# showlab/VideoSwap

Measured on AMD Instinct MI355X. Metric: denoised frames/sec, 16-frame 512x512 clip @ 50 DDIM steps (end to end: inversion + CFG sampling), higher is better.
Workload: dtype f16; 1 GPU; BASELINE.json configs[1]: 16-frame 512x512 clip, SD-1.5 UNet3D + AnimateDiff motion modules, 50-step DDIM inversion (B=1) + 50-step CFG-7.5 DDIM sampling (B=2), 1 clip per GPU per step; launch=eager, parallelism=clip-parallel x1

## Files before the change

### videoswap_amd/csrc/gemm.hip

```cpp
#include "gemm_common.h"
#include "prof.h"
#include <algorithm>
#include <cstdlib>
#include <stdlib.h>
#include <string.h>

using namespace vsxg;

static long tile_tune() { return vsxg::gemm_option("tile_tune"); }
static long force_tile() { return tile_tune() & 15; }
static bool tune_deep() { return (tile_tune() & 16) != 0; }
static int tune_splits() { return (int)((tile_tune() >> 8) & 15); }

namespace {


#ifdef VSX_GEMM_TIMING
#define TSTAMP(i) do { const long t_now = (long)clock64(); t_seg[i] += t_now - t_last; t_last = t_now; } while (0)
#else
#define TSTAMP(i) do { } while (0)
#endif

template <int BM, int BN, int WAVES_M, int WAVES_N, bool SWAP, int NSTAGE>
__global__ __launch_bounds__(WAVES_M* WAVES_N * 64) void gemm_kernel(const GemmParams p) {
    constexpr int PREFETCH = NSTAGE - 1;
    constexpr int NW = WAVES_M * WAVES_N;
    constexpr int WM = BM / WAVES_M, WN = BN / WAVES_N;
    constexpr int TM = WM / 32, TN = WN / 32;
    constexpr int A_BLKS = BM / 8, B_BLKS = BN / 8;
    static_assert(A_BLKS % NW == 0, "A blocks must split evenly over the waves");
    constexpr int GA = A_BLKS / NW;
    constexpr int GB_LO = B_BLKS / NW, GB_HI = (B_BLKS + NW - 1) / NW;
    constexpr int N_HI = B_BLKS - GB_LO * NW;
    constexpr int STAGE = (BM + BN) * 128;

    extern __shared__ __attribute__((aligned(16))) unsigned char smem[];

    const int tid = threadIdx.x;
    const int lane = tid & 63;
    const int wave = __builtin_amdgcn_readfirstlane(tid >> 6);
    const int wr = wave / WAVES_N, wc = wave % WAVES_N;
    const int l31 = lane & 31, hi = lane >> 5;
#ifdef VSX_GEMM_TIMING
    const long t_begin = (long)clock64();
#endif

    int tile_n, tile_m, split;
    if (p.xcd_gm > 0) {
        const int xcd = blockIdx.x & 7, local = blockIdx.x >> 3;
        const int gm = p.xcd_gm;
        const int RB = p.tiles_m / gm;
        const int CB = (p.tiles_n * (p.splitk > 1 ? p.splitk : 1)) / (8 / gm);
        const int lr = local % RB;
        const int np = (xcd / gm) * CB + local / RB;
        tile_m = (xcd % gm) * RB + lr;
        tile_n = np % p.tiles_n;
        split = np / p.tiles_n;
    } else {
        int wg = blockIdx.x;
        const int nwg = gridDim.x, q = nwg >> 3, r = nwg & 7;
        const int xcd = wg & 7, local = wg >> 3;
        wg = (xcd < r ? xcd * (q + 1) : r * (q + 1) + (xcd - r) * q) + local;
        tile_n = wg % p.tiles_n;
        tile_m = wg / p.tiles_n;
        split = p.splitk > 1 ? (int)blockIdx.z : 0;
    }
    const long m0 = (long)tile_m * BM;
    const long n0 = p.geglu ? (long)tile_n * (BN / 2) : (long)tile_n * BN;

    const int z = (p.splitk > 1 || p.xcd_gm > 0) ? 0 : (int)blockIdx.z;
    const int z0 = z / p.batch1, z1 = z - z0 * p.batch1;
    const half_t* Ab = p.A + z0 * p.a_bs0 + z1 * p.a_bs1;
    const half_t* Bb = p.B + z0 * p.b_bs0 + z1 * p.b_bs1;

    constexpr int OOB_OFF = (int)0x80000000;
    const int lrow = lane >> 3;
    const int pslot = lane & 7;
    const int kofs_e = (pslot ^ (lrow >> 1)) * 8;
    const int kofs_o = (pslot ^ (4 | (lrow >> 1))) * 8;

    const __amdgpu_buffer_rsrc_t rsrcA =
        __builtin_amdgcn_make_buffer_rsrc(const_cast<half_t*>(Ab), 0, (int)p.a_bytes, 0x00020000);
    const __amdgpu_buffer_rsrc_t rsrcA2 =
        __builtin_amdgcn_make_buffer_rsrc(const_cast<half_t*>(p.A2 ? p.A2 : p.A), 0, (int)p.a2_bytes, 0x00020000);
    const __amdgpu_buffer_rsrc_t rsrcB =
        __builtin_amdgcn_make_buffer_rsrc(const_cast<half_t*>(Bb), 0, (int)p.b_bytes, 0x00020000);

// ... 9 lines not shown
        a_ok[i] = m < p.M;
        a_h0[i] = 0; a_w0[i] = 0; a_ibase[i] = 0;
        a_kofs[i] = ((wave * GA + i) & 1) ? kofs_o : kofs_e;
        va[i] = a_ok[i] ? (int)((m * p.lda + a_kofs[i]) * 2) : OOB_OFF;
        if (p.a_mode == 1) {
            const long hw = (long)p.Ho * p.Wo;
            const long mm = a_ok[i] ? m : 0;
            const int img = (int)(mm / hw);
            const int rem = (int)(mm - (long)img * hw);
            const int ho = rem / p.Wo;
            a_h0[i] = ho * p.stride - pad;
            a_w0[i] = (rem - ho * p.Wo) * p.stride - pad;
            a_ibase[i] = img * Hs;
        }
    }
    const int gbw = wave < N_HI ? GB_HI : GB_LO;
    const int b_blk0 = wave < N_HI ? wave * GB_HI : N_HI * GB_HI + (wave - N_HI) * GB_LO;
    int vb[GB_HI], b_kofs[GB_HI];
#pragma unroll
    for (int j = 0; j < GB_HI; ++j) {
        const int jr = (b_blk0 + j) * 8 + lrow;
        b_kofs[j] = ((b_blk0 + j) & 1) ? kofs_o : kofs_e;
        long n;
        bool ok;
        if (p.geglu) {
            const long oc = n0 + (jr >> 5) * 16 + (jr & 15);
            ok = oc < p.N;
            n = oc + ((jr & 16) ? p.N : 0);
        } else {
            n = n0 + jr;
            ok = n < p.N;
        }
        vb[j] = (ok && j < gbw) ? (int)((n * p.ldb + b_kofs[j]) * 2) : OOB_OFF;
    }

    const int Ctot = p.C1 + p.C2;
    const int nk = (int)((p.K + BK - 1) / BK);
    const int ktail_from = (int)(p.K - (long)(nk - 1) * BK);
    const bool fast_tap = p.a_mode == 1 && (Ctot % BK == 0) && (p.C1 % BK == 0);
    const int kt_begin = split * p.nk_per;
    const int kt_end = p.splitk > 1 ? min(nk, kt_begin + p.nk_per) : nk;
    int t_kh = 0, t_kw = 0, t_c = 0;
    bool t_second = false, t_dirty = true;
    if (fast_tap && kt_begin > 0) {
        const int k0 = kt_begin * BK;
        const int tap = k0 / Ctot, rem = k0 - tap * Ctot;
        t_kh = tap / p.ks;
        t_kw = tap - t_kh * p.ks;
        t_second = rem >= p.C1;
        t_c = t_second ? rem - p.C1 : rem;
    }

    unsigned char* i_sb = smem;
    bool i_tail = false, i_second = false;
    int i_soffA = 0, i_soffB = 0;
    auto issue_prep = [&](int kt, int stage) {
        unsigned char* sb = smem + stage * STAGE;
        const bool last_tail = (kt == nk - 1) && ktail_from < BK;
        int soffA = kt * (BK * 2), soffB = kt * (BK * 2);
        bool second = false;
        if (p.a_mode == 1) {
            if (fast_tap) {
                if (t_dirty) {
                    const int cs = t_second ? p.C2 : p.C1;
#pragma unroll
                    for (int i = 0; i < GA; ++i) {
                        const int hh = a_h0[i] + t_kh, ww = a_w0[i] + t_kw;
                        const bool ok = a_ok[i] && (unsigned)hh < (unsigned)p.H && (unsigned)ww < (unsigned)p.W;
                        const int hsrc = p.ups ? (hh >> 1) : hh, wsrc = p.ups ? (ww >> 1) : ww;
                        va[i] = ok ? (((a_ibase[i] + hsrc) * Ws + wsrc) * cs + a_kofs[i]) * 2 : OOB_OFF;
                    }
                    t_dirty = false;
                }
                second = t_second;
                soffA = t_c * 2;
                t_c += BK;
                if (t_c >= (t_second ? p.C2 : p.C1)) {
                    t_c = 0;
                    t_dirty = true;
                    if (!t_second && p.C2 > 0) {
                        t_second = true;
                    } else {
                        t_second = false;
                        if (++t_kw == p.ks) { t_kw = 0; ++t_kh; }
                    }
                }
            } else {
#pragma unroll
                for (int i = 0; i < GA; ++i) {
                    const long k = (long)kt * BK + a_kofs[i];
                    const int kk = k < p.K ? (int)k : 0;
                    const int tap = kk / Ctot;
                    const int ci = kk - tap * Ctot;
                    const int kh = tap / p.ks, kw = tap - kh * p.ks;
                    const int hh = a_h0[i] + kh, ww = a_w0[i] + kw;
                    const bool ok = a_ok[i] && k < p.K && (unsigned)hh < (unsigned)p.H && (unsigned)ww < (unsigned)p.W;
                    const int hsrc = p.ups ? (hh >> 1) : hh, wsrc = p.ups ? (ww >> 1) : ww;
                    va[i] = ok ? (((a_ibase[i] + hsrc) * Ws + wsrc) * p.C1 + ci) * 2 : OOB_OFF;
                }
                soffA = 0;
            }
        }
        i_sb = sb; i_tail = last_tail; i_second = second; i_soffA = soffA; i_soffB = soffB;
    };
    constexpr int NPIECE = GA + GB_HI;
    bool i_on = true;
    bool i_gate = true;
    auto issue_piece = [&](const int q) {
        if (!(i_on && i_gate)) return;
        if (q < GA) {
            const int qi = q < GA ? q : 0;
            const int v = (i_tail && a_kofs[qi] >= ktail_from) ? OOB_OFF : va[qi];
            lptr_t dst = (lptr_t)(i_sb + (wave * GA + q) * 1024);
            if (i_second)
                __builtin_amdgcn_raw_ptr_buffer_load_lds(rsrcA2, dst, 16, v, i_soffA, 0, 0);
            else
                __builtin_amdgcn_raw_ptr_buffer_load_lds(rsrcA, dst, 16, v, i_soffA, 0, 0);
        } else {
            const int j = q - GA;
            if (j < gbw) {
                const int jj = j < GB_HI ? j : 0;
                const int v = (i_tail && b_kofs[jj] >= ktail_from) ? OOB_OFF : vb[jj];
                __builtin_amdgcn_raw_ptr_buffer_load_lds(rsrcB, (lptr_t)(i_sb + BM * 128 + (b_blk0 + j) * 1024), 16, v,
                                                         i_soffB, 0, 0);
            }
        }
    };
    auto issue = [&](int kt, int stage) {
        issue_prep(kt, stage);
        i_on = true;
        i_gate = true;
#pragma unroll
        for (int q = 0; q < NPIECE; ++q) issue_piece(q);
    };

    constexpr int NACC = SWAP ? TN : TM, MACC = SWAP ? TM : TN;
    f16v acc[NACC][MACC];
#pragma unroll
    for (int i = 0; i < NACC; ++i)
#pragma unroll
        for (int j = 0; j < MACC; ++j)
#pragma unroll
            for (int r = 0; r < 16; ++r) acc[i][j][r] = 0.f;

    const int swz = (l31 >> 1) & 7;
    const int a_row = (wr * WM + l31) * 128;
    const int b_row = BM * 128 + (wc * WN + l31) * 128;
    int offs[4];
#pragma unroll
    for (int ks = 0; ks < 4; ++ks) offs[ks] = ((ks * 2 + hi) ^ swz) * 16;

    const int nloc = kt_end - kt_begin;
#pragma unroll
    for (int s = 0; s < PREFETCH; ++s)
        if (s < nloc) issue(kt_begin + s, s);

    constexpr bool PRE_RES = SWAP && (NW <= 8) && (TM * TN <= 5);
    constexpr int NRES = TM * TN * 2;
    h4 rpre[PRE_RES ? TM * TN * 4 : 1];
    const half_t* Rb0 = p.residual ? p.residual + z0 * p.r_bs0 + z1 * p.r_bs1 : nullptr;
    const bool pre_res = PRE_RES && Rb0 != nullptr && p.vec4 && !p.geglu && p.splitk <= 1;
    const bool res_late = pre_res && p.rvec8 && (int)n0 + BN <= (int)p.N;
    bool r_inflight = false;
    auto issue_residual = [&]() {
        if constexpr (PRE_RES) {
#pragma unroll
            for (int i = 0; i < TM; ++i) {
                const unsigned m = (unsigned)min((int)m0 + wr * WM + i * 32 + l31, (int)p.M - 1);
#pragma unroll
                for (int j = 0; j < TN; ++j)
#pragma unroll
                    for (int a = 0; a < 2; ++a) {
                        const int nc = (int)n0 + wc * WN + j * 32 + 16 * a + 8 * hi;
                        const uint4 v = *reinterpret_cast<const uint4*>(Rb0 + m * (unsigned)p.ldr + nc);
                        rpre[(i * TN + j) * 4 + 2 * a] = __builtin_bit_cast(h4, make_uint2(v.x, v.y));
                        rpre[(i * TN + j) * 4 + 2 * a + 1] = __builtin_bit_cast(h4, make_uint2(v.z, v.w));
                    }
            }
        }
    };
    const bool res_early = (p.pp_flags & TILE_RES_EARLY) != 0;
    const int kt_r = res_early ? 0 : max(nloc - 1 - PREFETCH, 0);
    bool r_loaded = false;
    auto wait_slab = [&](const int kt) {
        const int later = min(nloc - 1 - kt, PREFETCH - 1);
        if (PRE_RES && r_inflight) {
            if (wave < N_HI) {
                constexpr int G = GA + GB_HI;
                if (PREFETCH >= 3 && later >= 2) wait_vmcnt<2 * G + NRES>();
                else if (PREFETCH >= 2 && later == 1) wait_vmcnt<G + NRES>();
                else wait_vmcnt<NRES>();
            } else {
                constexpr int G = GA + GB_LO;
                if (PREFETCH >= 3 && later >= 2) wait_vmcnt<2 * G + NRES>();
                else if (PREFETCH >= 2 && later == 1) wait_vmcnt<G + NRES>();
                else wait_vmcnt<NRES>();
            }
            return;
        }
        if (wave < N_HI) {
            constexpr int G = GA + GB_HI;
            if (PREFETCH >= 3 && later >= 2) wait_vmcnt<2 * G>();
            else if (PREFETCH >= 2 && later == 1) wait_vmcnt<G>();
            else wait_vmcnt<0>();
        } else {
            constexpr int G = GA + GB_LO;
            if (PREFETCH >= 3 && later >= 2) wait_vmcnt<2 * G>();
            else if (PREFETCH >= 2 && later == 1) wait_vmcnt<G>();
            else wait_vmcnt<0>();
        }
    };
    auto ldfrag = [&](const unsigned char* sb, const int off, h8 (&af)[TM], h8 (&bf)[TN]) {
#pragma unroll
        for (int i = 0; i < TM; ++i) af[i] = *reinterpret_cast<const h8*>(sb + a_row + i * 4096 + off);
#pragma unroll
        for (int j = 0; j < TN; ++j) bf[j] = *reinterpret_cast<const h8*>(sb + b_row + j * 4096 + off);
    };
    auto mma = [&](const h8 (&af)[TM], const h8 (&bf)[TN]) {
#pragma unroll
        for (int i = 0; i < TM; ++i)
#pragma unroll
            for (int j = 0; j < TN; ++j) {
                if constexpr (SWAP)
                    acc[j][i] = __builtin_amdgcn_mfma_f32_32x32x16_f16(bf[j], af[i], acc[j][i], 0, 0, 0);
                else
                    acc[i][j] = __builtin_amdgcn_mfma_f32_32x32x16_f16(af[i], bf[j], acc[i][j], 0, 0, 0);
            }
    };

    auto mma_issue = [&](const h8 (&af)[TM], const h8 (&bf)[TN], const bool gate) {
        i_gate = gate;
#pragma unroll
        for (int i = 0; i < TM; ++i)
#pragma unroll
            for (int j = 0; j < TN; ++j) {
                if constexpr (SWAP)
                    acc[j][i] = __builtin_amdgcn_mfma_f32_32x32x16_f16(bf[j], af[i], acc[j][i], 0, 0, 0);
                else
                    acc[i][j] = __builtin_amdgcn_mfma_f32_32x32x16_f16(af[i], bf[j], acc[i][j], 0, 0, 0);
                if (i * TN + j < NPIECE) issue_piece(i * TN + j);
            }
#pragma unroll
        for (int q = TM * TN; q < NPIECE; ++q) issue_piece(q);
    };

#ifdef VSX_GEMM_TIMING
    long t_seg[4] = {0, 0, 0, 0}, t_last = 0, t_loop0 = 0;
#endif
    constexpr bool PIPE = (NW <= 8) && (TM * TN < 10);
    if constexpr (PIPE) {
        h8 af0[TM], bf0[TN], af1[TM], bf1[TN];
        wait_slab(0);
        __builtin_amdgcn_s_barrier();
        if (PREFETCH < nloc) issue(kt_begin + PREFETCH, PREFETCH & (NSTAGE - 1));
        ldfrag(smem, offs[0], af0, bf0);
        const bool late = NW >= 8 && wave >= NW / 2;
        i_on = false;
#ifdef VSX_GEMM_TIMING
        t_last = t_loop0 = (long)clock64();
#endif
        for (int kt = 0; kt + 1 < nloc; ++kt) {
            const unsigned char* sb = smem + (kt & (NSTAGE - 1)) * STAGE;
            ldfrag(sb, offs[1], af1, bf1);
            __builtin_amdgcn_sched_barrier(0);
            mma_issue(af0, bf0, late);
            __builtin_amdgcn_sched_barrier(0);
            if constexpr (PRE_RES) {
                if (res_late && kt == kt_r) {
                    issue_residual();
                    VSX_VMEM_NOTE(NRES);
                    r_inflight = !res_early;
                    r_loaded = true;
                }
                __builtin_amdgcn_sched_barrier(0);
            }
            ldfrag(sb, offs[2], af0, bf0);
            __builtin_amdgcn_sched_barrier(0);
            mma(af1, bf1);
            __builtin_amdgcn_sched_barrier(0);
            ldfrag(sb, offs[3], af1, bf1);
            __builtin_amdgcn_sched_barrier(0);
            mma(af0, bf0);
            __builtin_amdgcn_sched_barrier(0);
            TSTAMP(0);
            wait_slab(kt + 1);
            __builtin_amdgcn_s_waitcnt(0xC07F);
            TSTAMP(1);
            __builtin_amdgcn_s_barrier();
            TSTAMP(2);
            i_on = kt + 1 + PREFETCH < nloc;
            if (i_on) issue_prep(kt_begin + kt + 1 + PREFETCH, (kt + 1 + PREFETCH) & (NSTAGE - 1));
            ldfrag(smem + ((kt + 1) & (NSTAGE - 1)) * STAGE, offs[0], af0, bf0);
            __builtin_amdgcn_sched_barrier(0);
            mma_issue(af1, bf1, !late);
            __builtin_amdgcn_sched_barrier(0);
            TSTAMP(3);
        }
        if (nloc > 0) {
            const unsigned char* sb = smem + ((nloc - 1) & (NSTAGE - 1)) * STAGE;
            ldfrag(sb, offs[1], af1, bf1);
            mma(af0, bf0);
            ldfrag(sb, offs[2], af0, bf0);
            mma(af1, bf1);
            ldfrag(sb, offs[3], af1, bf1);
            mma(af0, bf0);
            mma(af1, bf1);
        }
    } else {
        const bool late16 = NW >= 16 && ((wave >> 2) & 1);
#ifdef VSX_GEMM_TIMING
        t_last = t_loop0 = (long)clock64();
#endif
        for (int kt = 0; kt < nloc; ++kt) {
            wait_slab(kt);
            TSTAMP(1);
            __builtin_amdgcn_s_barrier();
            TSTAMP(2);
            i_on = kt + PREFETCH < nloc;
            i_gate = true;
            if (i_on) issue_prep(kt_begin + kt + PREFETCH, (kt + PREFETCH) & (NSTAGE - 1));
            if (!late16) {
#pragma unroll
                for (int q = 0; q < NPIECE; ++q) issue_piece(q);
            }
            TSTAMP(3);
            const unsigned char* sb = smem + (kt & (NSTAGE - 1)) * STAGE;
#pragma unroll
            for (int ks = 0; ks < 4; ++ks) {
                h8 af[TM], bf[TN];
                ldfrag(sb, offs[ks], af, bf);
                mma(af, bf);
                if (ks == 0 && late16) {
#pragma unroll
                    for (int q = 0; q < NPIECE; ++q) issue_piece(q);
                }
            }
            TSTAMP(0);
        }
    }

#ifdef VSX_GEMM_TIMING
    long* const t_out = p.ws && p.splitk <= 1 ? reinterpret_cast<long*>(p.ws) + ((long)blockIdx.x * NW + wave) * 8 : nullptr;
    if (lane == 0 && t_out) {
        for (int k = 0; k < 4; ++k) t_out[k] = t_seg[k];
        t_out[4] = t_begin; t_out[5] = t_loop0; t_out[6] = (long)clock64();
    }
#define TSTAMP_END() do { asm volatile("s_waitcnt vmcnt(0)" ::: "memory"); if (lane == 0 && t_out) t_out[7] = (long)clock64(); } while (0)
#else
#define TSTAMP_END() do { } while (0)
#endif
    half_t* Cb = p.C + z0 * p.c_bs0 + z1 * p.c_bs1;
    const half_t* Rb = p.residual ? p.residual + z0 * p.r_bs0 + z1 * p.r_bs1 : nullptr;
    const int Mi = (int)p.M, Ni = (int)p.N;
    const int ldc = (int)p.ldc, ldr = (int)p.ldr;
    const int mb = (int)m0, nb0 = (int)n0;

    if constexpr (SWAP) {
        if (p.splitk > 1) {
            float* wsl = p.ws + (size_t)split * (size_t)Mi * (size_t)Ni;
#pragma unroll
            for (int i = 0; i < TM; ++i) {
                const int m = mb + wr * WM + i * 32 + l31;
                if (m >= Mi) continue;
#pragma unroll
                for (int j = 0; j < TN; ++j)
#pragma unroll
                    for (int g = 0; g < 4; ++g) {
                        const int nb = nb0 + wc * WN + j * 32 + 8 * g + 4 * hi;
                        if (nb + 3 < Ni) {
                            f4v o;
#pragma unroll
                            for (int e = 0; e < 4; ++e) o[e] = acc[j][i][4 * g + e] * p.alpha;
                            *reinterpret_cast<f4v*>(wsl + (size_t)m * Ni + nb) = o;
                        }
                    }
            }
            return;
        }
        constexpr bool PRE_BIAS = (NW <= 8) && (TM * TN <= 5);
        h4 bpre[PRE_BIAS ? TN : 1][4];
        const bool pre_bias = PRE_BIAS && p.bias != nullptr && p.vec8 && !p.geglu;
        if constexpr (PRE_BIAS) {
            if (pre_bias) {
#pragma unroll
                for (int j = 0; j < TN; ++j)
#pragma unroll
                    for (int g = 0; g < 4; ++g) {
                        const int nb = nb0 + wc * WN + j * 32 + 8 * g + 4 * hi;
                        bpre[j][g] = nb + 3 < Ni ? *reinterpret_cast<const h4*>(p.bias + nb) : h4{};
                    }
            }
        }
#pragma unroll
        for (int i = 0; i < TM; ++i) {
            const int m = mb + wr * WM + i * 32 + l31;
// ... 269 lines not shown
    if (p.residual) {
        const h4 b = *reinterpret_cast<const h4*>(p.residual + (size_t)m * p.ldr + nb);
#pragma unroll
        for (int e = 0; e < 4; ++e) acc[e] += (float)b[e];
    }
    h4 pk;
#pragma unroll
    for (int e = 0; e < 4; ++e) pk[e] = (half_t)acc[e];
    *reinterpret_cast<h4*>(p.C + (size_t)m * p.ldc + nb) = pk;
}

inline int plan_splitk(const vsx_gemm_desc* d, long tiles, bool eligible) {
    const long nk = (d->K + BK - 1) / BK;
    if (eligible && tune_splits() > 0) return tune_splits() <= nk ? tune_splits() : (int)nk;
    if (!eligible || tiles >= 160) return 1;
    int s = (int)((256 + tiles - 1) / tiles);
    if (s > 8) s = 8;
    while (s > 1 && nk / s < 12) --s;
    return s;
}

int plan_xcd_grid(const GemmParams& p, const long tiles_m, const int bm, const int bn, const long nbatch) {
    if (nbatch != 1 || gemm_option("xcd_walk") == 0) return 0;
    const int splits = p.splitk > 1 ? p.splitk : 1;
    const long np_total = (long)p.tiles_n * splits;
    if ((tiles_m * np_total) % 8 != 0 || tiles_m * np_total < 16) return 0;
    const long nk = (p.K + BK - 1) / BK;
    const double kslice = (double)(splits > 1 ? (long)p.nk_per * BK : nk * BK);
    const double taps = p.a_mode == 1 ? (double)(p.ks * p.ks) / (double)(p.stride * p.stride) : 1.0;
    const double a_panel = (double)bm * kslice * 2.0 / (taps < 1.0 ? 1.0 : taps);
    const double b_panel = (double)bn * kslice * 2.0;
    auto cost = [&](const int gm) -> double {
        const int gn = 8 / gm;
        if (tiles_m % gm != 0 || np_total % gn != 0) return -1.0;
        const long RB = tiles_m / gm, CB = np_total / gn;
        long nsp = 1;
        for (int b = 0; b < gn; ++b) {
            const long lo = b * CB, hi = lo + CB - 1;
            nsp = std::max(nsp, hi / p.tiles_n - lo / p.tiles_n + 1);
        }
        return (double)(RB * nsp) * a_panel + (double)CB * b_panel;
    };
    const double legacy = (tiles_m % 8 == 0) ? cost(8)
                                             : (double)((tiles_m + 7) / 8 + 1) * splits * a_panel + (double)np_total * b_panel;
    int best = 0;
    double best_cost = legacy;
    for (int gm = 4; gm >= 1; gm >>= 1) {
        const double c = cost(gm);
        if (c >= 0.0 && c < 0.95 * best_cost) { best = gm; best_cost = c; }
    }
    return best;
}

template <int BM, int BN, int WAVES_M, int WAVES_N, bool SWAP, int NSTAGE>
int launch(GemmParams& p, long tiles_m, long nbatch, hipStream_t stream) {
    constexpr size_t smem = (size_t)NSTAGE * (BM + BN) * 128;
    static_assert(smem <= 160 * 1024, "LDS ring exceeds 160 KiB");
    static bool attr_set = false;
    if (!attr_set) {
        hipError_t e = hipFuncSetAttribute(reinterpret_cast<const void*>(&gemm_kernel<BM, BN, WAVES_M, WAVES_N, SWAP, NSTAGE>),
                                           hipFuncAttributeMaxDynamicSharedMemorySize, (int)smem);
        if (e != hipSuccess) return vsx_fail(VSX_E_LAUNCH, "gemm: hipFuncSetAttribute: %s", hipGetErrorString(e));
        attr_set = true;
    }
    p.pp_flags = (int)(gemm_option("pp_sched") & TILE_RES_EARLY);
    p.tiles_m = (int)tiles_m;
    p.xcd_gm = plan_xcd_grid(p, tiles_m, BM, BN, nbatch);
    dim3 grid((unsigned)(tiles_m * p.tiles_n), 1, (unsigned)(p.splitk > 1 ? p.splitk : nbatch));
    if (p.xcd_gm > 0) grid = dim3((unsigned)(tiles_m * p.tiles_n * (p.splitk > 1 ? p.splitk : 1)), 1, 1);
    hipLaunchKernelGGL((gemm_kernel<BM, BN, WAVES_M, WAVES_N, SWAP, NSTAGE>), grid, dim3(WAVES_M * WAVES_N * 64), smem,
                       stream, p);
    return vsx_check_launch("vsx_gemm_f16");
}

template <int BM, int BN, int WAVES_M, int WAVES_N>
int launch_tile(GemmParams& p, long M, long cols, long nbatch, hipStream_t stream, bool deep = false) {
    p.tiles_n = (int)((cols + BN - 1) / BN);
    const long tiles_m = (M + BM - 1) / BM;
    constexpr int NST = ((BM + BN) * 128 * 4 <= 96 * 1024) ? 4 : 2;
    if constexpr (BM == 128 && BN == 160) {
        if (deep && p.c_mode != 1) return launch<BM, BN, WAVES_M, WAVES_N, true, 4>(p, tiles_m, nbatch, stream);
    }
    if (p.c_mode == 1) return launch<BM, BN, WAVES_M, WAVES_N, false, NST>(p, tiles_m, nbatch, stream);
    return launch<BM, BN, WAVES_M, WAVES_N, true, NST>(p, tiles_m, nbatch, stream);
}


int pp_mode() { return (int)gemm_option("gemm_pp"); }

enum GemmFamily { GEMM_WS, GEMM_PP256, GEMM_PP128, GEMM_TILE };
enum GemmRefusal { PLAN_OK = 0, PLAN_SUBPIXEL_OFF_PP, PLAN_ROWSTATS_PARTS };

struct GemmPlan {
    GemmFamily family;
    int BM, BN, WAVES_M, WAVES_N;
    bool deep;
    bool forced;
    long nbatch;
    int splits, nk_per;
    long stat_parts;
    int64_t workspace_bytes;
    GemmRefusal refused;
};

int fill_conv_params(const vsx_gemm_desc* d, GemmParams& p, const long nbatch) {
    VSX_REQUIRE(nbatch == 1, VSX_E_UNSUPPORTED, "gemm: conv mode does not take a batch");
    VSX_REQUIRE(d->ks == 1 || d->ks == 3, VSX_E_UNSUPPORTED, "gemm: conv kernel size %ld", (long)d->ks);
    VSX_REQUIRE(d->stride == 1 || d->stride == 2, VSX_E_UNSUPPORTED, "gemm: conv stride %ld", (long)d->stride);
    VSX_REQUIRE(d->C1 > 0 && d->C1 % 8 == 0 && d->C2 >= 0 && d->C2 % 8 == 0, VSX_E_BADSHAPE,
                "gemm: conv channels must be multiples of 8 (C1=%ld C2=%ld)", (long)d->C1, (long)d->C2);
    VSX_REQUIRE((d->C2 == 0) == (d->A2 == nullptr), VSX_E_BADSHAPE, "gemm: A2/C2 mismatch");
    VSX_REQUIRE(d->A2 == nullptr || vsx_aligned16(d->A2), VSX_E_BADSHAPE, "gemm: A2 must be 16-byte aligned");
    VSX_REQUIRE(d->K == d->ks * d->ks * (d->C1 + d->C2), VSX_E_BADSHAPE, "gemm: conv K mismatch");
    VSX_REQUIRE(d->C2 == 0 || (d->C1 % 64 == 0 && d->C2 % 64 == 0), VSX_E_UNSUPPORTED,
                "gemm: a two-source conv needs both channel counts to be multiples of 64 (one K slab)");
    VSX_REQUIRE(d->H > 0 && d->W > 0, VSX_E_BADSHAPE, "gemm: conv H/W");
    VSX_REQUIRE(!d->upsample || (d->H % 2 == 0 && d->W % 2 == 0), VSX_E_BADSHAPE, "gemm: upsample needs even H/W");
    p.H = (int)d->H; p.W = (int)d->W; p.C1 = (int)d->C1; p.C2 = (int)d->C2;
    p.ks = (int)d->ks; p.stride = (int)d->stride; p.ups = d->upsample ? 1 : 0;
    const bool subpix = d->upsample == 2;
    if (subpix) {
        VSX_REQUIRE(d->ks == 3 && d->stride == 1 && d->C2 == 0 && d->C1 % 64 == 0 && d->pad_lo < 0 && d->pad_hi < 0 &&
                        !d->rowvec && !d->residual && !d->geglu && d->c_mode == 0 && !d->rowscale && !d->rowstats,
                    VSX_E_UNSUPPORTED, "gemm: the sub-pixel form takes a single-source 3x3 stride-1 convolution with a bias only");
        VSX_REQUIRE(d->M % 4 == 0, VSX_E_BADSHAPE, "gemm: sub-pixel form: M must be a multiple of 4");
        p.ups = 0;
        p.H = (int)d->H / 2;
        p.W = (int)d->W / 2;
        p.sp_Mc = (int)(d->M / 4);
        p.K = 4 * d->C1;
    }
    const bool sym = d->pad_lo < 0 && d->pad_hi < 0;
    VSX_REQUIRE(sym || (d->pad_lo >= 0 && d->pad_hi >= 0 && d->pad_lo < d->ks && d->pad_hi < d->ks), VSX_E_BADSHAPE,
                "gemm: conv padding (%ld, %ld) for kernel size %ld", (long)d->pad_lo, (long)d->pad_hi, (long)d->ks);
    const int pad_lo = sym ? p.ks / 2 : (int)d->pad_lo, pad_hi = sym ? p.ks / 2 : (int)d->pad_hi;
    p.pad = pad_lo;
// ... 211 lines not shown
    else if (is_tile<128, 128, 2, 2>(plan)) rc = launch_tile<128, 128, 2, 2>(p, p.M, cols, nbatch, stream);
    else if (is_tile<64, 128, 2, 2>(plan)) rc = launch_tile<64, 128, 2, 2>(p, p.M, cols, nbatch, stream);
    else if (is_tile<64, 64, 2, 2>(plan)) rc = launch_tile<64, 64, 2, 2>(p, p.M, cols, nbatch, stream);
    else return vsx_fail(VSX_E_UNSUPPORTED, "gemm: no tile kernel %d x %d", plan.BM, plan.BN);
    if (plan.splits > 1 && rc == VSX_OK) {
        const long quads = p.M * (p.N / 4);
        hipLaunchKernelGGL(splitk_reduce_kernel, dim3((unsigned)((quads + 255) / 256)), dim3(256), 0, stream, p);
        rc = vsx_check_launch("vsx_gemm_f16 (split-K reduce)");
    }
    return rc;
}

}

extern "C" int vsx_gemm_f16(const vsx_gemm_desc* d, vsx_stream_t stream_) {
    hipStream_t stream = (hipStream_t)stream_;
    GemmParams p;
    int rc = fill_params(d, p);
    if (rc != VSX_OK || d->M == 0) return rc;
    const GemmPlan plan = plan_gemm(*d, p, false);
    VSX_REQUIRE(plan.refused != PLAN_ROWSTATS_PARTS, VSX_E_UNSUPPORTED,
                "gemm: rowstats with %ld parts, but this launch writes %ld (ask vsx_gemm_rowstats_parts first)",
                (long)d->rowstats_parts, plan.stat_parts);
    VSX_REQUIRE(plan.refused != PLAN_SUBPIXEL_OFF_PP, VSX_E_UNSUPPORTED,
                "gemm: the sub-pixel form runs on the persistent kernel only (enough tiles, rows per class a multiple of the tile)");
    if (d->rowstats != nullptr) {
        VSX_REQUIRE(vsx_aligned16(d->rowstats), VSX_E_BADSHAPE, "gemm: rowstats must be 16-byte aligned");
        p.rowstats = (float*)d->rowstats;
        p.rowstats_parts = (int)plan.stat_parts;
    }
    if (plan.forced || plan.splits > 1) p.ws = (float*)d->workspace;
    const long sample = prof_begin(stream);
    if (sample == PROF_FAILED) return VSX_E_LAUNCH;
    rc = run_plan(plan, p, stream);
    if (sample >= 0) {
        double flop, bytes;
        gemm_work(*d, p, &flop, &bytes);
        prof_end(sample, stream, flop, bytes);
    }
    return rc;
}

extern "C" int64_t vsx_gemm_rowstats_parts(const vsx_gemm_desc* d) {
    GemmParams p;
    if (!d || d->M <= 0 || fill_params(d, p) != VSX_OK) return 0;
    return plan_gemm(*d, p, false).stat_parts;
}

extern "C" int64_t vsx_gemm_workspace(const vsx_gemm_desc* d) {
    GemmParams p;
    if (!d || d->M <= 0 || fill_params(d, p) != VSX_OK) return 0;
    return plan_gemm(*d, p, true).workspace_bytes;
}
```

### videoswap_amd/csrc/gemm_pp.hip

```cpp
#include "gemm_common.h"

#include <stdlib.h>

#ifndef VSX_PP_ABLATE
#define VSX_PP_ABLATE 0
#endif

namespace vsxg {
#ifdef VSX_GEMM_TIMING
__device__ long* g_pp_dbg = nullptr;
#endif
namespace {

typedef const __attribute__((address_space(4))) GemmParams* kparams_t;
typedef float f2v __attribute__((ext_vector_type(2)));

__device__ __forceinline__ int fresh_lane(const int lane_hint) {
    int l = lane_hint;
    asm volatile("v_mbcnt_lo_u32_b32 %0, -1, 0\n\tv_mbcnt_hi_u32_b32 %0, -1, %0" : "=v"(l));
    return l;
}

__device__ __forceinline__ kparams_t kernarg_params() {
    kparams_t kp = (kparams_t)__builtin_amdgcn_kernarg_segment_ptr();
// ... 598 lines not shown
            const int col = (row0 + l31) & wmask;
            const bool edge = (c_kw == 0 && col == 0) || (c_kw == 2 && col == wmask);
            aoff[i] = edge ? ZERO_OFF : base + i * 4096;
        }
    };
    auto ldfrag = [&](const int slot_off, const int ks_) {
        int ks = ks_;
        asm volatile("" : "+s"(ks));
#pragma unroll
        for (int i = 0; i < TM; ++i) {
            if constexpr (ashift) af[i] = *reinterpret_cast<const h8*>(smem + (aoff[i] ^ (ks * 32)));
            else af[i] = *reinterpret_cast<const h8*>(smem + slot_off + ((a_addr ^ (ks * 32)) + i * 4096));
        }
#pragma unroll
        for (int j = 0; j < TN; ++j)
            bf[j] = *reinterpret_cast<const h8*>(smem + slot_off + ((b_addr ^ (ks * 32)) + j * 4096));
    };
    auto mma = [&]() {
#pragma unroll
        for (int i = 0; i < TM; ++i)
#pragma unroll
            for (int j = 0; j < TN; ++j)
                acc[j][i] = __builtin_amdgcn_mfma_f32_32x32x16_f16(bf[j], af[i], acc[j][i], 0, 0, 0);
    };
    auto mma_first = [&]() {
        const f16v zero = {};
#pragma unroll
        for (int i = 0; i < TM; ++i)
#pragma unroll
            for (int j = 0; j < TN; ++j)
                acc[j][i] = __builtin_amdgcn_mfma_f32_32x32x16_f16(bf[j], af[i], zero, 0, 0, 0);
    };
    auto lgkm0 = [&]() { __builtin_amdgcn_s_waitcnt(0xC07F); };
    auto bar = [&]() {
        __builtin_amdgcn_sched_barrier(0);
        __builtin_amdgcn_s_barrier();
        __builtin_amdgcn_sched_barrier(0);
    };

    if constexpr (ashift) {
        if (tid < 32) reinterpret_cast<float*>(smem + ZERO_OFF)[tid] = 0.f;
        lgkm0();
    }
    slab_prep();
    issue_range(0, NPIECE);
    wait_vmcnt<0>();
    bar();
    if (G == 1) bar();

    int c_g = 0;
#ifdef VSX_GEMM_TIMING
    long t_seg[3] = {0, 0, 0}, t_last = (long)__builtin_amdgcn_s_memtime();
#define PPSTAMP(i) do { const long t_now = (long)__builtin_amdgcn_s_memtime(); t_seg[i] += t_now - t_last; t_last = t_now; } while (0)
#else
#define PPSTAMP(i) do { } while (0)
#endif
    for (int c_t = 0; c_t < n_my; ++c_t) {
        for (int kt = 0; kt < nk; ++kt, ++c_g) {
            const int so = (c_g & 1) * STAGE;
            i_on = i_t < n_my;
            if (i_on) slab_prep();
            if constexpr (ashift) {
                if (kt == 0) { c_kw = 0; c_aslot = c_g & 1; }
                else if (++c_kw == 3) { c_kw = 0; c_aslot ^= 1; }
                shared_a_setup();
            }
            ldfrag(so, 0);
            __builtin_amdgcn_sched_barrier(0);
            issue_range(0, CUT1);
            lgkm0();
            bar();
            __builtin_amdgcn_s_setprio(1);
            if (kt == 0) mma_first(); else mma();
            __builtin_amdgcn_s_setprio(0);
            bar();
            ldfrag(so, 1);
            __builtin_amdgcn_sched_barrier(0);
            issue_range(CUT1, CUT2);
            lgkm0();
            bar();
            __builtin_amdgcn_s_setprio(1);
            mma();
            __builtin_amdgcn_s_setprio(0);
            bar();
            ldfrag(so, 2);
            __builtin_amdgcn_sched_barrier(0);
            issue_range(CUT2, NPIECE);
            lgkm0();
            bar();
            __builtin_amdgcn_s_setprio(1);
            mma();
            __builtin_amdgcn_s_setprio(0);
            bar();
            ldfrag(so, 3);
            __builtin_amdgcn_sched_barrier(0);
            if (G == 1) wait_vmcnt<0>();
            lgkm0();
            bar();
            __builtin_amdgcn_s_setprio(1);
            mma();
            __builtin_amdgcn_s_setprio(0);
            __builtin_amdgcn_sched_barrier(0);
            if (G == 0) wait_vmcnt<0>();
            if (kt + 1 < nk) bar();
        }
        if (G == 0) bar();
        PPSTAMP(0);
        {
            const int tile = tile0 + c_t * wgx;
            int tile_n, tile_m;
            tile_coords(tile, tiles_n, tiles_m, blocked, tile_m, tile_n);
            const int n0 = geglu ? tile_n * (BN / 2) : tile_n * BN;
            const int stg_off = wave < NFIT ? ((c_g - 1) & 1) * STAGE + wave * EP_BYTES
                                            : 2 * STAGE + (wave - NFIT) * EP_BYTES;
            constexpr int PD = (EPI & EPI_LN) ? 2 : ((CONV || (EPI & EPI_STATS)) ? 3 : 4);
            epilogue_pp<TM, EPI, PD, CONV == 3>(acc, reinterpret_cast<float*>(smem + stg_off), tile_m * BM + wr * WM, n0 + wc * WN,
                                 n0 + wc * TN * 16, lane);
        }
        __builtin_amdgcn_sched_barrier(0);
        lgkm0();
        PPSTAMP(1);
        bar();
        if (G == 1) bar();
        PPSTAMP(2);
    }
#ifdef VSX_GEMM_TIMING
    if (lane == 0 && g_pp_dbg) {
        long* o_dbg = g_pp_dbg + ((long)blockIdx.x * 8 + wave) * 4;
        o_dbg[0] = t_seg[0]; o_dbg[1] = t_seg[1]; o_dbg[2] = t_seg[2]; o_dbg[3] = n_my;
    }
#endif
    if (G == 0) bar();
}

template <int TM, int CONV, int EPI>
int launch_one(const GemmParams& p, hipStream_t stream) {
    constexpr size_t stage = (size_t)(128 * TM + 320) * 128;
    constexpr size_t smem = 2 * stage + (8 - stage / EP_BYTES) * EP_BYTES + (CONV == 2 ? 128 : 0);
    static_assert(smem <= 160 * 1024, "LDS budget");
    static bool attr_set = false;
    if (!attr_set) {
        hipError_t e = hipFuncSetAttribute(reinterpret_cast<const void*>(&gemm_pp_kernel<TM, CONV, EPI>),
                                           hipFuncAttributeMaxDynamicSharedMemorySize, (int)smem);
        if (e != hipSuccess) return vsx_fail(VSX_E_LAUNCH, "gemm_pp: hipFuncSetAttribute: %s", hipGetErrorString(e));
        attr_set = true;
    }
    static int n_cu = 0;
    if (n_cu == 0) {
        int dev = 0;
        hipDeviceProp_t prop;
        if (hipGetDevice(&dev) != hipSuccess || hipGetDeviceProperties(&prop, dev) != hipSuccess)
            return vsx_fail(VSX_E_LAUNCH, "gemm_pp: cannot query the device");
        n_cu = prop.multiProcessorCount > 0 ? prop.multiProcessorCount : 256;
    }
    const int grid = p.tiles_total < n_cu ? p.tiles_total : n_cu;
    hipLaunchKernelGGL((gemm_pp_kernel<TM, CONV, EPI>), dim3((unsigned)grid), dim3(512), smem, stream, p, p.tiles_total);
    return vsx_check_launch("vsx_gemm_f16 (persistent)");
}


constexpr int WS_NST = 3;
constexpr int WS_XST = 32 * 640;
constexpr int WS_R0 = WS_NST * WS_XST;
constexpr int WS_RST = 32 * 640;
constexpr int WS_S0 = WS_R0 + 2 * WS_RST;
template <int NW>
struct WsGeo {
    static constexpr int COLS = 320 / NW, NB = COLS / 32, LPR = COLS / 8, RPP = 64 / LPR, PASSES = 32 / RPP;
    static constexpr int PITCH = NB * 32 + 4;
    static constexpr int SCST = NW == 5 ? EP_CONST : 32 * PITCH;
    static constexpr int EPW = NW == 5 ? EP_BYTES : (SCST + 160 + COLS) * 4;
    static constexpr int RS0 = WS_S0 + NW * EPW;
    static constexpr int LDS = RS0 + 2 * 1024;
    static constexpr int WREG = 3 * COLS * 128;
    static_assert(LDS <= 160 * 1024 && WS_XST + NW * WREG <= LDS, "LDS budget of the weight-stationary kernel");
};

template <int EPI, int NW>
__global__ __launch_bounds__(NW * 64) void gemm_ws320_kernel(const GemmParams p_unused, const int nblocks, const int nslices) {
    typedef WsGeo<NW> G_;
    constexpr int COLS = G_::COLS, NB = G_::NB, LPR = G_::LPR, RPP = G_::RPP, PASSES = G_::PASSES, XP = 20 / NW;
    constexpr bool ADD = (EPI & EPI_ADD) != 0, STATS = (EPI & EPI_STATS) != 0, LN = (EPI & EPI_LN) != 0;
    constexpr int LDT = XP + (ADD ? PASSES : 0) + (LN ? 1 : 0), ST = STATS ? 2 * PASSES : PASSES;
    constexpr int OOB_OFF = (int)0x80000000;
    extern __shared__ __attribute__((aligned(16))) unsigned char smem[];
    kparams_t p = kernarg_params();
    const int tid = threadIdx.x;
    const int lane = tid & 63;
    const int wave = __builtin_amdgcn_readfirstlane(tid >> 6);
    const int l31 = lane & 31, hi = lane >> 5;
    const int lrow = lane >> 3, pslot = lane & 7;
    const unsigned lda2 = (unsigned)p->lda * 2u, ldb = (unsigned)p->ldb;
    const int xcd = blockIdx.x & 7, local = blockIdx.x >> 3;
    const int slice = local % nslices, grp = local / nslices;
    const int ngroups = ((int)gridDim.x >> 3) / nslices * 8;
    const int chain = grp * 8 + xcd;
    const int ncol_s = 320 * slice;
    const bool is_rowvec = ADD && p->residual == nullptr;
    const unsigned ldr2 = is_rowvec ? (unsigned)p->N * 2u : (unsigned)p->ldr * 2u;
    const unsigned rpv = is_rowvec ? (unsigned)p->rows_per_vec : 1u;

    const __amdgpu_buffer_rsrc_t rsrcA =
        __builtin_amdgcn_make_buffer_rsrc(const_cast<half_t*>(p->A), 0, (int)p->a_bytes, 0x00020000);
    const unsigned r_rows = is_rowvec ? (unsigned)((p->M + (long)rpv - 1) / (long)rpv) : (unsigned)p->M;
    const __amdgpu_buffer_rsrc_t rsrcR = __builtin_amdgcn_make_buffer_rsrc(
        const_cast<half_t*>(ADD ? (is_rowvec ? p->rowvec : p->residual) : p->A), 0,
        ADD ? (int)((r_rows - 1u) * ldr2 + (unsigned)p->N * 2u) : 0, 0x00020000);
    const int vx_e = (int)((unsigned)lrow * lda2) + (pslot ^ (lrow >> 1)) * 16;
// ... 305 lines not shown
```

### videoswap_amd/csrc/options.cpp

```cpp
#include "options.h"

#include <stdlib.h>
#include <string.h>

#include "common.h"

namespace vsxg {
namespace {
struct Option { const char* name; const char* env; long value; bool init; };
Option g_options[] = {{"gemm_pp", "VSX_GEMM_PP", 1, false}, {"pp_sched", "VSX_PP_SCHED", 0, false},
                      {"tile_tune", "VSX_TUNE_TILE", 0, false}, {"xcd_walk", "VSX_XCD_WALK", 1, false},
                      {"attn_qb", "VSX_ATTN_QB", 0, false}, {"temporal_out", "VSX_TEMPORAL_OUT", 0, false},
                      {"attn_o16", "VSX_ATTN_O16", 0, false}, {"gn_fuse", "VSX_GN_FUSE", 0, false},
                      {"gemm_ws", "VSX_GEMM_WS", 1, false}, {"ws_waves", "VSX_WS_WAVES", 10, false}};
Option* find_option(const char* name) {
    for (auto& o : g_options)
        if (strcmp(o.name, name) == 0) {
            if (!o.init) {
                const char* e = getenv(o.env);
                if (e) o.value = atol(e);
                o.init = true;
            }
            return &o;
        }
    return nullptr;
}
}
long gemm_option(const char* name) {
    Option* o = find_option(name);
    return o ? o->value : 0;
}
}

extern "C" int vsx_set_option(const char* name, int64_t value) {
    auto* o = name ? vsxg::find_option(name) : nullptr;
    if (!o) return vsx_fail(VSX_E_BADSHAPE, "vsx_set_option: unknown option '%s'", name ? name : "(null)");
    o->value = (long)value;
    return VSX_OK;
}
```

Before: 4.156 frames/s.

## Add asymmetric LDS ring that prefetches B one slab ahead of A

```diff
diff --git a/videoswap_amd/csrc/gemm.hip b/videoswap_amd/csrc/gemm.hip
--- a/videoswap_amd/csrc/gemm.hip
+++ b/videoswap_amd/csrc/gemm.hip
@@ -16,14 +16,19 @@
 
 
 #ifdef VSX_GEMM_TIMING
+__device__ long* g_tile_dbg = nullptr;
 #define TSTAMP(i) do { const long t_now = (long)clock64(); t_seg[i] += t_now - t_last; t_last = t_now; } while (0)
 #else
 #define TSTAMP(i) do { } while (0)
 #endif
 
-template <int BM, int BN, int WAVES_M, int WAVES_N, bool SWAP, int NSTAGE>
+#ifndef VSX_BA_SLACK
+#define VSX_BA_SLACK 0
+#endif
+template <int BM, int BN, int WAVES_M, int WAVES_N, bool SWAP, int NSTAGE, bool B3 = false>
 __global__ __launch_bounds__(WAVES_M* WAVES_N * 64) void gemm_kernel(const GemmParams p) {
     constexpr int PREFETCH = NSTAGE - 1;
+    static_assert(!B3 || (NSTAGE == 2 && SWAP), "the asymmetric ring extends the two-slot ring");
     constexpr int NW = WAVES_M * WAVES_N;
     constexpr int WM = BM / WAVES_M, WN = BN / WAVES_N;
     constexpr int TM = WM / 32, TN = WN / 32;
@@ -33,6 +38,9 @@
     constexpr int GB_LO = B_BLKS / NW, GB_HI = (B_BLKS + NW - 1) / NW;
     constexpr int N_HI = B_BLKS - GB_LO * NW;
     constexpr int STAGE = (BM + BN) * 128;
+    auto a_slot = [](const int s) { return B3 ? (s & 1) * (BM * 128) : (s & (NSTAGE - 1)) * STAGE; };
+    auto b_slot = [](const int s) { return B3 ? 2 * BM * 128 + (s % 3) * (BN * 128) : 0; };
+    constexpr int B_ROWS_AT = B3 ? 0 : BM * 128;
 
     extern __shared__ __attribute__((aligned(16))) unsigned char smem[];
 
@@ -148,12 +156,14 @@
     }
 
     unsigned char* i_sb = smem;
-    bool i_tail = false, i_second = false;
+    unsigned char* i_sbB = smem;
+    bool i_tail = false, i_tailB = false, i_second = false, i_onB = true;
     int i_soffA = 0, i_soffB = 0;
-    auto issue_prep = [&](int kt, int stage) {
-        unsigned char* sb = smem + stage * STAGE;
+    auto issue_prep = [&](int kt, int sl) {
+        unsigned char* sb = smem + (B3 ? a_slot(sl) : sl * STAGE);
+        const int ktb = B3 ? kt + 1 : kt, slb = B3 ? sl + 1 : sl;
         const bool last_tail = (kt == nk - 1) && ktail_from < BK;
-        int soffA = kt * (BK * 2), soffB = kt * (BK * 2);
+        int soffA = kt * (BK * 2), soffB = ktb * (BK * 2);
         bool second = false;
         if (p.a_mode == 1) {
             if (fast_tap) {
@@ -198,6 +208,11 @@
             }
         }
         i_sb = sb; i_tail = last_tail; i_second = second; i_soffA = soffA; i_soffB = soffB;
+        if constexpr (B3) {
+            i_sbB = smem + b_slot(slb);
+            i_tailB = (ktb == nk - 1) && ktail_from < BK;
+            i_onB = ktb < kt_end;
+        }
     };
     constexpr int NPIECE = GA + GB_HI;
     bool i_on = true;
@@ -214,16 +229,16 @@
                 __builtin_amdgcn_raw_ptr_buffer_load_lds(rsrcA, dst, 16, v, i_soffA, 0, 0);
         } else {
             const int j = q - GA;
-            if (j < gbw) {
+            if (j < gbw && (!B3 || i_onB)) {
                 const int jj = j < GB_HI ? j : 0;
-                const int v = (i_tail && b_kofs[jj] >= ktail_from) ? OOB_OFF : vb[jj];
-                __builtin_amdgcn_raw_ptr_buffer_load_lds(rsrcB, (lptr_t)(i_sb + BM * 128 + (b_blk0 + j) * 1024), 16, v,
+                const int v = ((B3 ? i_tailB : i_tail) && b_kofs[jj] >= ktail_from) ? OOB_OFF : vb[jj];
+                __builtin_amdgcn_raw_ptr_buffer_load_lds(rsrcB, (lptr_t)((B3 ? i_sbB : i_sb) + B_ROWS_AT + (b_blk0 + j) * 1024), 16, v,
                                                          i_soffB, 0, 0);
             }
         }
     };
-    auto issue = [&](int kt, int stage) {
-        issue_prep(kt, stage);
+    auto issue = [&](int kt, int sl) {
+        issue_prep(kt, sl);
         i_on = true;
         i_gate = true;
 #pragma unroll
@@ -241,12 +256,22 @@
 
     const int swz = (l31 >> 1) & 7;
     const int a_row = (wr * WM + l31) * 128;
-    const int b_row = BM * 128 + (wc * WN + l31) * 128;
+    const int b_row = B_ROWS_AT + (wc * WN + l31) * 128;
     int offs[4];
 #pragma unroll
     for (int ks = 0; ks < 4; ++ks) offs[ks] = ((ks * 2 + hi) ^ swz) * 16;
 
     const int nloc = kt_end - kt_begin;
+    if constexpr (B3) {
+        if (nloc > 0) {
+            i_sbB = smem + b_slot(0);
+            i_soffB = kt_begin * (BK * 2);
+            i_tailB = (kt_begin == nk - 1) && ktail_from < BK;
+            i_onB = true; i_on = true; i_gate = true;
+#pragma unroll
+            for (int q = GA; q < NPIECE; ++q) issue_piece(q);
+        }
+    }
 #pragma unroll
     for (int s = 0; s < PREFETCH; ++s)
         if (s < nloc) issue(kt_begin + s, s);
@@ -279,6 +304,16 @@
     const int kt_r = res_early ? 0 : max(nloc - 1 - PREFETCH, 0);
     bool r_loaded = false;
     auto wait_slab = [&](const int kt) {
+        if constexpr (B3) {
+            constexpr int GBW = GB_LO + VSX_BA_SLACK;
+            static_assert(N_HI == 0, "every wave issues the same number of B pieces");
+            if (kt + 1 < nloc) {
+                if (PRE_RES && r_inflight) wait_vmcnt<GBW + NRES>(); else wait_vmcnt<GBW>();
+            } else {
+                if (PRE_RES && r_inflight) wait_vmcnt<NRES>(); else wait_vmcnt<0>();
+            }
+            return;
+        }
         const int later = min(nloc - 1 - kt, PREFETCH - 1);
         if (PRE_RES && r_inflight) {
             if (wave < N_HI) {
@@ -306,11 +341,11 @@
             else wait_vmcnt<0>();
         }
     };
-    auto ldfrag = [&](const unsigned char* sb, const int off, h8 (&af)[TM], h8 (&bf)[TN]) {
+    auto ldfrag = [&](const unsigned char* sb, const int off, h8 (&af)[TM], h8 (&bf)[TN], const unsigned char* sbb = nullptr) {
 #pragma unroll
         for (int i = 0; i < TM; ++i) af[i] = *reinterpret_cast<const h8*>(sb + a_row + i * 4096 + off);
 #pragma unroll
-        for (int j = 0; j < TN; ++j) bf[j] = *reinterpret_cast<const h8*>(sb + b_row + j * 4096 + off);
+        for (int j = 0; j < TN; ++j) bf[j] = *reinterpret_cast<const h8*>((B3 ? sbb : sb) + b_row + j * 4096 + off);
     };
     auto mma = [&](const h8 (&af)[TM], const h8 (&bf)[TN]) {
 #pragma unroll
@@ -344,20 +379,22 @@
     long t_seg[4] = {0, 0, 0, 0}, t_last = 0, t_loop0 = 0;
 #endif
     constexpr bool PIPE = (NW <= 8) && (TM * TN < 10);
+    static_assert(!B3 || PIPE, "the asymmetric ring lives in the register-pipelined loop");
     if constexpr (PIPE) {
         h8 af0[TM], bf0[TN], af1[TM], bf1[TN];
         wait_slab(0);
         __builtin_amdgcn_s_barrier();
-        if (PREFETCH < nloc) issue(kt_begin + PREFETCH, PREFETCH & (NSTAGE - 1));
-        ldfrag(smem, offs[0], af0, bf0);
+        if (PREFETCH < nloc) issue(kt_begin + PREFETCH, B3 ? PREFETCH : PREFETCH & (NSTAGE - 1));
+        ldfrag(smem, offs[0], af0, bf0, smem + b_slot(0));
         const bool late = NW >= 8 && wave >= NW / 2;
         i_on = false;
 #ifdef VSX_GEMM_TIMING
         t_last = t_loop0 = (long)clock64();
 #endif
         for (int kt = 0; kt + 1 < nloc; ++kt) {
-            const unsigned char* sb = smem + (kt & (NSTAGE - 1)) * STAGE;
-            ldfrag(sb, offs[1], af1, bf1);
+            const unsigned char* sb = smem + a_slot(kt);
+            const unsigned char* sbb = B3 ? smem + b_slot(kt) : nullptr;
+            ldfrag(sb, offs[1], af1, bf1, sbb);
             __builtin_amdgcn_sched_barrier(0);
             mma_issue(af0, bf0, late);
             __builtin_amdgcn_sched_barrier(0);
@@ -370,11 +407,11 @@
                 }
                 __builtin_amdgcn_sched_barrier(0);
             }
-            ldfrag(sb, offs[2], af0, bf0);
+            ldfrag(sb, offs[2], af0, bf0, sbb);
             __builtin_amdgcn_sched_barrier(0);
             mma(af1, bf1);
             __builtin_amdgcn_sched_barrier(0);
-            ldfrag(sb, offs[3], af1, bf1);
+            ldfrag(sb, offs[3], af1, bf1, sbb);
             __builtin_amdgcn_sched_barrier(0);
             mma(af0, bf0);
             __builtin_amdgcn_sched_barrier(0);
@@ -385,20 +422,21 @@
             __builtin_amdgcn_s_barrier();
             TSTAMP(2);
             i_on = kt + 1 + PREFETCH < nloc;
-            if (i_on) issue_prep(kt_begin + kt + 1 + PREFETCH, (kt + 1 + PREFETCH) & (NSTAGE - 1));
-            ldfrag(smem + ((kt + 1) & (NSTAGE - 1)) * STAGE, offs[0], af0, bf0);
+            if (i_on) issue_prep(kt_begin + kt + 1 + PREFETCH, B3 ? kt + 1 + PREFETCH : (kt + 1 + PREFETCH) & (NSTAGE - 1));
+            ldfrag(smem + a_slot(kt + 1), offs[0], af0, bf0, B3 ? smem + b_slot(kt + 1) : nullptr);
             __builtin_amdgcn_sched_barrier(0);
             mma_issue(af1, bf1, !late);
             __builtin_amdgcn_sched_barrier(0);
             TSTAMP(3);
         }
         if (nloc > 0) {
-            const unsigned char* sb = smem + ((nloc - 1) & (NSTAGE - 1)) * STAGE;
-            ldfrag(sb, offs[1], af1, bf1);
+            const unsigned char* sb = smem + a_slot(nloc - 1);
+            const unsigned char* sbb = B3 ? smem + b_slot(nloc - 1) : nullptr;
+            ldfrag(sb, offs[1], af1, bf1, sbb);
             mma(af0, bf0);
-            ldfrag(sb, offs[2], af0, bf0);
+            ldfrag(sb, offs[2], af0, bf0, sbb);
             mma(af1, bf1);
-            ldfrag(sb, offs[3], af1, bf1);
+            ldfrag(sb, offs[3], af1, bf1, sbb);
             mma(af0, bf0);
             mma(af1, bf1);
         }
@@ -436,7 +474,8 @@
     }
 
 #ifdef VSX_GEMM_TIMING
-    long* const t_out = p.ws && p.splitk <= 1 ? reinterpret_cast<long*>(p.ws) + ((long)blockIdx.x * NW + wave) * 8 : nullptr;
+    long* const t_out = g_tile_dbg ? g_tile_dbg + (((long)blockIdx.z * gridDim.x + blockIdx.x) * NW + wave) * 8
+                        : (p.ws && p.splitk <= 1 ? reinterpret_cast<long*>(p.ws) + ((long)blockIdx.x * NW + wave) * 8 : nullptr);
     if (lane == 0 && t_out) {
         for (int k = 0; k < 4; ++k) t_out[k] = t_seg[k];
         t_out[4] = t_begin; t_out[5] = t_loop0; t_out[6] = (long)clock64();
@@ -812,13 +851,13 @@
     return best;
 }
 
-template <int BM, int BN, int WAVES_M, int WAVES_N, bool SWAP, int NSTAGE>
+template <int BM, int BN, int WAVES_M, int WAVES_N, bool SWAP, int NSTAGE, bool B3 = false>
 int launch(GemmParams& p, long tiles_m, long nbatch, hipStream_t stream) {
-    constexpr size_t smem = (size_t)NSTAGE * (BM + BN) * 128;
+    constexpr size_t smem = B3 ? (size_t)(2 * BM + 3 * BN) * 128 : (size_t)NSTAGE * (BM + BN) * 128;
     static_assert(smem <= 160 * 1024, "LDS ring exceeds 160 KiB");
     static bool attr_set = false;
     if (!attr_set) {
-        hipError_t e = hipFuncSetAttribute(reinterpret_cast<const void*>(&gemm_kernel<BM, BN, WAVES_M, WAVES_N, SWAP, NSTAGE>),
+        hipError_t e = hipFuncSetAttribute(reinterpret_cast<const void*>(&gemm_kernel<BM, BN, WAVES_M, WAVES_N, SWAP, NSTAGE, B3>),
                                            hipFuncAttributeMaxDynamicSharedMemorySize, (int)smem);
         if (e != hipSuccess) return vsx_fail(VSX_E_LAUNCH, "gemm: hipFuncSetAttribute: %s", hipGetErrorString(e));
         attr_set = true;
@@ -828,7 +867,7 @@
     p.xcd_gm = plan_xcd_grid(p, tiles_m, BM, BN, nbatch);
     dim3 grid((unsigned)(tiles_m * p.tiles_n), 1, (unsigned)(p.splitk > 1 ? p.splitk : nbatch));
     if (p.xcd_gm > 0) grid = dim3((unsigned)(tiles_m * p.tiles_n * (p.splitk > 1 ? p.splitk : 1)), 1, 1);
-    hipLaunchKernelGGL((gemm_kernel<BM, BN, WAVES_M, WAVES_N, SWAP, NSTAGE>), grid, dim3(WAVES_M * WAVES_N * 64), smem,
+    hipLaunchKernelGGL((gemm_kernel<BM, BN, WAVES_M, WAVES_N, SWAP, NSTAGE, B3>), grid, dim3(WAVES_M * WAVES_N * 64), smem,
                        stream, p);
     return vsx_check_launch("vsx_gemm_f16");
 }
@@ -842,6 +881,9 @@
         if (deep && p.c_mode != 1) return launch<BM, BN, WAVES_M, WAVES_N, true, 4>(p, tiles_m, nbatch, stream);
     }
     if (p.c_mode == 1) return launch<BM, BN, WAVES_M, WAVES_N, false, NST>(p, tiles_m, nbatch, stream);
+    if constexpr (BM == 128 && BN == 320) {
+        if (gemm_option("b_ahead") == 2) return launch<BM, BN, WAVES_M, WAVES_N, true, NST, true>(p, tiles_m, nbatch, stream);
+    }
     return launch<BM, BN, WAVES_M, WAVES_N, true, NST>(p, tiles_m, nbatch, stream);
 }
 
@@ -1159,3 +1201,9 @@
     if (!d || d->M <= 0 || fill_params(d, p) != VSX_OK) return 0;
     return plan_gemm(*d, p, true).workspace_bytes;
 }
+
+#ifdef VSX_GEMM_TIMING
+extern "C" int vsx_tile_debug_buffer(void* buf) {
+    return hipMemcpyToSymbol(HIP_SYMBOL(g_tile_dbg), &buf, sizeof(buf)) == hipSuccess ? 0 : 1;
+}
+#endif
diff --git a/videoswap_amd/csrc/gemm_pp.hip b/videoswap_amd/csrc/gemm_pp.hip
--- a/videoswap_amd/csrc/gemm_pp.hip
+++ b/videoswap_amd/csrc/gemm_pp.hip
@@ -674,8 +674,13 @@
 #ifdef VSX_GEMM_TIMING
     long t_seg[3] = {0, 0, 0}, t_last = (long)__builtin_amdgcn_s_memtime();
 #define PPSTAMP(i) do { const long t_now = (long)__builtin_amdgcn_s_memtime(); t_seg[i] += t_now - t_last; t_last = t_now; } while (0)
+    long t_w[2] = {0, 0}, t_w0 = 0;
+#define PPWAIT_BEGIN() do { t_w0 = (long)__builtin_amdgcn_s_memtime(); } while (0)
+#define PPWAIT_ADD(i) do { const long t_now = (long)__builtin_amdgcn_s_memtime(); t_w[i] += t_now - t_w0; t_w0 = t_now; } while (0)
 #else
 #define PPSTAMP(i) do { } while (0)
+#define PPWAIT_BEGIN() do { } while (0)
+#define PPWAIT_ADD(i) do { } while (0)
 #endif
     for (int c_t = 0; c_t < n_my; ++c_t) {
         for (int kt = 0; kt < nk; ++kt, ++c_g) {
@@ -716,15 +721,18 @@
             bar();
             ldfrag(so, 3);
             __builtin_amdgcn_sched_barrier(0);
-            if (G == 1) wait_vmcnt<0>();
+            if (G == 1) { PPWAIT_BEGIN(); wait_vmcnt<0>(); PPWAIT_ADD(0); }
             lgkm0();
+            if (G == 1) PPWAIT_BEGIN();
             bar();
+            if (G == 1) PPWAIT_ADD(1);
             __builtin_amdgcn_s_setprio(1);
             mma();
             __builtin_amdgcn_s_setprio(0);
             __builtin_amdgcn_sched_barrier(0);
-            if (G == 0) wait_vmcnt<0>();
+            if (G == 0) { PPWAIT_BEGIN(); wait_vmcnt<0>(); PPWAIT_ADD(0); }
             if (kt + 1 < nk) bar();
+            if (G == 0) PPWAIT_ADD(1);
         }
         if (G == 0) bar();
         PPSTAMP(0);
@@ -748,8 +756,9 @@
     }
 #ifdef VSX_GEMM_TIMING
     if (lane == 0 && g_pp_dbg) {
-        long* o_dbg = g_pp_dbg + ((long)blockIdx.x * 8 + wave) * 4;
+        long* o_dbg = g_pp_dbg + ((long)blockIdx.x * 8 + wave) * 8;
         o_dbg[0] = t_seg[0]; o_dbg[1] = t_seg[1]; o_dbg[2] = t_seg[2]; o_dbg[3] = n_my;
+        o_dbg[4] = t_w[0]; o_dbg[5] = t_w[1];
     }
 #endif
     if (G == 0) bar();
@@ -775,7 +784,9 @@
             return vsx_fail(VSX_E_LAUNCH, "gemm_pp: cannot query the device");
         n_cu = prop.multiProcessorCount > 0 ? prop.multiProcessorCount : 256;
     }
-    const int grid = p.tiles_total < n_cu ? p.tiles_total : n_cu;
+    int grid = p.tiles_total < n_cu ? p.tiles_total : n_cu;
+    const long cap = gemm_option("pp_grid");
+    if (cap > 0 && cap < grid) grid = (int)cap;
     hipLaunchKernelGGL((gemm_pp_kernel<TM, CONV, EPI>), dim3((unsigned)grid), dim3(512), smem, stream, p, p.tiles_total);
     return vsx_check_launch("vsx_gemm_f16 (persistent)");
 }
diff --git a/videoswap_amd/csrc/options.cpp b/videoswap_amd/csrc/options.cpp
--- a/videoswap_amd/csrc/options.cpp
+++ b/videoswap_amd/csrc/options.cpp
@@ -12,7 +12,8 @@
                       {"tile_tune", "VSX_TUNE_TILE", 0, false}, {"xcd_walk", "VSX_XCD_WALK", 1, false},
                       {"attn_qb", "VSX_ATTN_QB", 0, false}, {"temporal_out", "VSX_TEMPORAL_OUT", 0, false},
                       {"attn_o16", "VSX_ATTN_O16", 0, false}, {"gn_fuse", "VSX_GN_FUSE", 0, false},
-                      {"gemm_ws", "VSX_GEMM_WS", 1, false}, {"ws_waves", "VSX_WS_WAVES", 10, false}};
+                      {"gemm_ws", "VSX_GEMM_WS", 1, false}, {"ws_waves", "VSX_WS_WAVES", 10, false},
+                      {"b_ahead", "VSX_B_AHEAD", 2, false}, {"pp_grid", "VSX_PP_GRID", 0, false}};
 Option* find_option(const char* name) {
     for (auto& o : g_options)
         if (strcmp(o.name, name) == 0) {
```

Measured after the change: 4.182 frames/s (median of 6 runs). Within noise of the previous version (+0.6%).
